# PSilvestre/Clonos

Hardware: AMD Instinct MI355X
Metric: determinants/sec decode+delta-slice (higher is better)
Workload: dtype u8

## Files before the change

### clonos_amd/build.py

```python
from __future__ import annotations

import os
import subprocess
import sys

HERE = os.path.dirname(os.path.abspath(__file__))
ROOT = os.path.dirname(HERE)
CSRC = os.path.join(HERE, "csrc")
LIB = os.path.join(HERE, "libclonos_engine.so")
SOURCES = [os.path.join(CSRC, "engine.cpp"), os.path.join(CSRC, "kernels.hip"), os.path.join(CSRC, "decode_fast.hip"),
           os.path.join(CSRC, "decode_fused.hip"), os.path.join(CSRC, "replay.hip"), os.path.join(CSRC, "encode.hip"),
           os.path.join(CSRC, "response.cpp"), os.path.join(CSRC, "digest.hip"),
           os.path.join(CSRC, "diff.hip")]
HEADERS = [
    os.path.join(CSRC, "kernels.h"),
    os.path.join(CSRC, "jser_device.h"),
    os.path.join(CSRC, "dev_common.h"),
    os.path.join(CSRC, "dev_slow.h"),
    os.path.join(CSRC, "jser_flat.h"),
    os.path.join(CSRC, "handoff.h"),
    os.path.join(CSRC, "digest.h"),
    os.path.join(CSRC, "diff.h"),
    os.path.join(ROOT, "include", "clonos_engine.h"),
]
ARCH = os.environ.get("CLONOS_OFFLOAD_ARCH", "gfx950")


def hipcc() -> str:
    for c in (os.environ.get("HIPCC"), "/opt/rocm/bin/hipcc", "hipcc"):
        if c and (os.path.isabs(c) and os.path.exists(c) or not os.path.isabs(c)):
            return c
    return "hipcc"


def needs_build() -> bool:
    if not os.path.exists(LIB):
        return True
    t = os.path.getmtime(LIB)
    return any(os.path.getmtime(p) > t for p in SOURCES + HEADERS)


def _compile_cmd(src: str, obj: str) -> list:
    return [
        hipcc(),
        "-x", "hip",
        f"--offload-arch={ARCH}",
        "-O3",
        "-std=c++17",
        "-fPIC",
        "-Wall",
        "-Wno-unused-function",
        "-Wno-unused-value",
        "-I", os.path.join(ROOT, "include"),
        "-c", src,
        "-o", obj,
    ]


def build(force: bool = False, verbose: bool = False) -> str:
    if not force and not needs_build():
        return LIB
    hdr_t = max(os.path.getmtime(h) for h in HEADERS)
    objs, procs = [], []
    for src in SOURCES:
        obj = os.path.join(CSRC, os.path.basename(src) + ".o")
        objs.append(obj)
        if not force and os.path.exists(obj) and os.path.getmtime(obj) > max(hdr_t, os.path.getmtime(src)):
            continue
        cmd = _compile_cmd(src, obj)
        if verbose:
            print(" ".join(cmd), flush=True)
        procs.append((src, subprocess.Popen(cmd)))
    bad = [src for src, p in procs if p.wait() != 0]
    if bad:
        raise RuntimeError(f"hipcc failed for {bad}")
    link = [hipcc(), f"--offload-arch={ARCH}", "-shared", "-fPIC", "-o", LIB] + objs
    if verbose:
        print(" ".join(link), flush=True)
    subprocess.run(link, check=True)
    return LIB


if __name__ == "__main__":
    build(force="--force" in sys.argv, verbose=True)
```

### clonos_amd/csrc/engine.cpp

```cpp
#include <hip/hip_runtime.h>
#include <sched.h>

#include <algorithm>
#include <chrono>
#include <condition_variable>
#include <cstdarg>
#include <cstdio>
#include <cstdlib>
#include <cstring>
#include <deque>
#include <functional>
#include <map>
#include <memory>
#include <atomic>
#include <mutex>
#include <string>
#include <thread>
#include <unordered_map>
#include <optional>
#include <vector>

#include "../../include/clonos_engine.h"
#include "diff.h"
#include "digest.h"
#include "kernels.h"

static_assert(sizeof(clg_delta_req) == 32, "clg_delta_req layout");
static_assert(sizeof(clg_diff) == 24, "clg_diff layout");

namespace {

thread_local std::string g_err;

int fail(int code, const char* fmt, ...) {
  char buf[512];
  va_list ap;
  va_start(ap, fmt);
  vsnprintf(buf, sizeof buf, fmt, ap);
  va_end(ap);
  g_err = buf;
  return code;
}

#define HIPCHK(x)                                                                                   \
  do {                                                                                              \
    hipError_t e_ = (x);                                                                            \
    if (e_ != hipSuccess) return fail(CLG_E_DEVICE, "%s failed: %s", #x, hipGetErrorString(e_)); \
  } while (0)

void note_launch_error(const char* what) {
  if (const char* m = clg::take_launch_error()) fail(CLG_E_DEVICE, "%s: %s", what, m);
}
#define CHK(x)                                          \
  do {                                                  \
    int r_ = (x);                                       \
    if (r_ != CLG_OK) {                                 \
      if (r_ == CLG_E_DEVICE) note_launch_error(#x);    \
      return r_;                                        \
    }                                                   \
  } while (0)

struct EpochStart {
  int64_t id;
  int32_t offset;
};
struct Consumer {
  std::shared_ptr<EpochStart> es;
  int32_t offset;
};

template <class T>
struct EpochAlloc {
  using value_type = T;
  EpochAlloc() = default;
  template <class U>
  EpochAlloc(const EpochAlloc<U>&) {}
  struct FreeList : std::vector<void*> {
    ~FreeList() {
      for (void* p : *this) ::operator delete(p);
    }
  };
  static FreeList& free_list() {
    static thread_local FreeList f;
    return f;
  }
  T* allocate(size_t n) {
    auto& f = free_list();
    if (n == 1 && !f.empty()) {
      void* p = f.back();
      f.pop_back();
      return static_cast<T*>(p);
    }
    return static_cast<T*>(::operator new(n * sizeof(T)));
  }
  void deallocate(T* p, size_t n) {
    auto& f = free_list();
    if (n == 1 && f.size() < (1u << 20)) f.push_back(p);
    else ::operator delete(p);
  }
  template <class U>
  bool operator==(const EpochAlloc<U>&) const { return true; }
  template <class U>
  bool operator!=(const EpochAlloc<U>&) const { return false; }
};

struct EpochEnt {
  int64_t id = 0;
  int32_t offset = 0;
  std::shared_ptr<EpochStart> shared;
};
class EpochMap {
 public:
  EpochEnt* begin() { return data(); }
  EpochEnt* end() { return data() + n_; }
  const EpochEnt* begin() const { return data(); }
  const EpochEnt* end() const { return data() + n_; }
  size_t size() const { return n_; }
  bool empty() const { return n_ == 0; }
  EpochEnt* find(int64_t k) {
    EpochEnt* it = lower(k);
    return it != end() && it->id == k ? it : end();
  }
  const EpochEnt* find(int64_t k) const { return const_cast<EpochMap*>(this)->find(k); }
  EpochEnt* emplace(int64_t k, int32_t offset) {
    EpochEnt* it = lower(k);
    if (it != end() && it->id == k) return it;
    const size_t i = size_t(it - begin());
    if (big_.empty() && n_ < kInline) {
      for (size_t j = n_; j > i; --j) inl_[j] = std::move(inl_[j - 1]);
      inl_[i] = EpochEnt{k, offset, nullptr};
    } else {
      if (big_.empty()) {
        big_.reserve(2 * kInline);
        for (uint32_t j = 0; j < n_; ++j) big_.push_back(std::move(inl_[j]));
        for (auto& x : inl_) x.shared.reset();
      }
      big_.insert(big_.begin() + long(i), EpochEnt{k, offset, nullptr});
    }
    ++n_;
    return begin() + i;
  }
  void erase_below(int64_t k) {
    const size_t d = size_t(lower(k) - begin());
    if (!d) return;
    if (big_.empty()) {
      for (size_t j = d; j < n_; ++j) inl_[j - d] = std::move(inl_[j]);
      for (size_t j = n_ - d; j < n_; ++j) inl_[j].shared.reset();
    } else {
      big_.erase(big_.begin(), big_.begin() + long(d));
    }
    n_ -= uint32_t(d);
  }
  void rebase(int32_t move) {
    for (EpochEnt& x : *this) {
      x.offset -= move;
      if (x.shared) x.shared->offset = x.offset;
    }
  }
  static std::shared_ptr<EpochStart> ref(EpochEnt& x) {
    if (!x.shared) x.shared = std::allocate_shared<EpochStart>(EpochAlloc<EpochStart>(), EpochStart{x.id, x.offset});
    return x.shared;
  }

 private:
  static constexpr uint32_t kInline = 2;
  EpochEnt* data() { return big_.empty() ? inl_ : big_.data(); }
  const EpochEnt* data() const { return big_.empty() ? inl_ : big_.data(); }
  EpochEnt* lower(int64_t k) {
    if (n_ == 0 || end()[-1].id < k) return end();
    return std::lower_bound(begin(), end(), k, [](const EpochEnt& a, int64_t b) { return a.id < b; });
  }
  uint32_t n_ = 0;
  EpochEnt inl_[kInline];
  std::vector<EpochEnt> big_;
};

class SegList {
 public:
// ... 154 lines not shown
  ~PinBuf() {
    if (p) hipHostFree(p);
  }
  template <class T>
  T* as() const { return static_cast<T*>(p); }
};

struct Stat {
  uint64_t launches = 0;
  double ms = 0;
  uint64_t bytes = 0;
};
struct PendingTiming {
  std::string name;
  hipEvent_t a, b;
  uint64_t bytes;
};

constexpr size_t kPoolGuard = 256;

constexpr uint32_t kLogStripes = 64;
struct alignas(64) Stripe {
  std::mutex m;
};
struct EngineLock {
  std::mutex m;
  std::atomic<std::thread::id> owner{};
  int depth = 0;
  Stripe stripe[kLogStripes];
  bool owned() const { return owner.load(std::memory_order_relaxed) == std::this_thread::get_id(); }
  void lock() {
    if (owned()) {
      ++depth;
      return;
    }
    m.lock();
    for (auto& s : stripe) s.m.lock();
    owner.store(std::this_thread::get_id(), std::memory_order_relaxed);
    depth = 1;
  }
  void unlock() {
    if (--depth == 0) {
      owner.store(std::thread::id(), std::memory_order_relaxed);
      for (uint32_t i = kLogStripes; i-- > 0;) stripe[i].m.unlock();
      m.unlock();
    }
  }
};
struct XGuard {
  EngineLock& l;
  explicit XGuard(EngineLock& l_) : l(l_) { l.lock(); }
  ~XGuard() { l.unlock(); }
};

class WorkPool {
 public:
  explicit WorkPool(unsigned n) : n_(n ? n : 1) {
    for (unsigned i = 1; i < n_; ++i) th_.emplace_back([this, i] { loop(i); });
  }
  ~WorkPool() {
    {
      std::lock_guard<std::mutex> g(mu_);
      stop_ = true;
    }
    cv_.notify_all();
    for (auto& t : th_) t.join();
  }
  unsigned size() const { return n_; }
  void run(const std::function<void(unsigned, unsigned)>& fn) {
    if (n_ == 1) {
      fn(0, 1);
      return;
    }
    {
      std::lock_guard<std::mutex> g(mu_);
      job_ = &fn;
      left_.store(n_ - 1, std::memory_order_relaxed);
      gen_.fetch_add(1, std::memory_order_release);
    }
    cv_.notify_all();
    fn(0, n_);
    while (left_.load(std::memory_order_acquire) != 0) std::this_thread::yield();
  }

 private:
  void loop(unsigned i) {
    uint64_t seen = 0;
    for (;;) {
      const auto t0 = std::chrono::steady_clock::now();
      while (gen_.load(std::memory_order_acquire) == seen &&
             std::chrono::steady_clock::now() - t0 < std::chrono::microseconds(50))
        std::this_thread::yield();
      const std::function<void(unsigned, unsigned)>* job;
      {
        std::unique_lock<std::mutex> g(mu_);
        cv_.wait(g, [&] { return stop_ || gen_.load(std::memory_order_acquire) != seen; });
        if (stop_) return;
        seen = gen_.load(std::memory_order_acquire);
        job = job_;
      }
      (*job)(i, n_);
      left_.fetch_sub(1, std::memory_order_acq_rel);
    }
  }
  unsigned n_;
  std::vector<std::thread> th_;
  std::mutex mu_;
  std::condition_variable cv_;
  std::atomic<uint64_t> gen_{0};
  std::atomic<unsigned> left_{0};
  const std::function<void(unsigned, unsigned)>* job_ = nullptr;
  bool stop_ = false;
};

}

namespace {
struct Mapped {
  uintptr_t host;
  uint64_t bytes;
  uintptr_t dev;
};
std::mutex g_map_mu;
std::vector<Mapped> g_mapped;
uintptr_t clg_mapped_device_address(const void* h, uint64_t n) {
  std::lock_guard<std::mutex> g(g_map_mu);
  for (const Mapped& m : g_mapped)
    if (uintptr_t(h) >= m.host && uintptr_t(h) < m.host + m.bytes && n <= m.host + m.bytes - uintptr_t(h))
      return m.dev + (uintptr_t(h) - m.host);
  return 0;
}
}

namespace clg_internal {
int set_error(int code, const char* msg) { return fail(code, "%s", msg); }
}

static long long env_num(const char* name, long long dflt, int base = 10) {
  const char* v = getenv(name);
  return v ? strtoll(v, nullptr, base) : dflt;
}
static std::string env_str(const char* name) {
  const char* v = getenv(name);
  return v ? v : "";
}
struct DevSwitches {
  bool robust_decode = env_str("CLONOS_DECODE") == "robust";
  bool small_decode = env_num("CLONOS_SMALL", 1) != 0;
  bool sidecar = env_num("CLONOS_SIDECAR", 1) != 0;
  bool keep_errors = env_num("CLONOS_KEEP_ERRORS", 1) != 0;
  uint32_t fused_perturb = uint32_t(env_num("CLONOS_FUSED_PERTURB", 0, 0));
  size_t jser_arena = getenv("CLONOS_JSER_ARENA") ? std::max<size_t>(256, size_t(env_num("CLONOS_JSER_ARENA", 0, 0))) : 0;
  int gather_prio = int(env_num("CLONOS_GATHER_PRIO", 1));
  int host_threads = int(env_num("CLONOS_HOST_THREADS", 16));
  int lean = int(env_num("CLONOS_LEAN", -1));
  int warm = int(env_num("CLONOS_WARM", -1));
  bool host_prof = getenv("CLONOS_HOST_PROF") != nullptr;
  bool fused_debug = getenv("CLONOS_FUSED_DEBUG") != nullptr;
  bool small_prof = getenv("CLONOS_SMALL_PROF") != nullptr;
  std::string scan_phases = env_str("CLONOS_SCAN_PHASES"), robust_phases = env_str("CLONOS_ROBUST_PHASES"),
              debug_dump = env_str("CLONOS_DEBUG_DUMP");
};

struct clg_engine {
  clg_config cfg{};
  const DevSwitches sw;
  hipStream_t stream = nullptr;
  void* pool_alloc = nullptr;
  uint8_t* pool = nullptr;
  std::vector<uint32_t> free_segs;
  clg::SideCar side{};
  void* side_alloc = nullptr;
  std::vector<uint32_t> seg_life;
  const clg::SideCar* side_arg() const { return side.hdr ? &side : nullptr; }
  uint32_t life_word(uint32_t seg, bool more) const { return (seg_life[seg] & 0x7FFFFFFFu) | (more ? 0x80000000u : 0u); }
  void* ifl_alloc = nullptr;
  uint8_t* ifl_pool = nullptr;
  uint32_t ifl_C = 0;
  std::vector<uint32_t> ifl_free;
  uint8_t* ifl_addr(uint32_t s) const { return ifl_pool + size_t(s) * ifl_C; }
  std::vector<Log> logs;
  std::vector<InFlight> ifls;
  std::map<IdKey, uint32_t> by_id;
  std::vector<Job> jobs;
  std::vector<uint32_t> dirty;
  EngineLock mu;
  std::mutex pool_mu;
  std::mutex dirty_mu;

  PinBuf h_stage, h_desc, h_sres, h_outs;
  static constexpr uint32_t kSlots = 1 + CLG_DECODE_MAX_INFLIGHT;
  PinBuf h_zres_s[kSlots], h_plan_s[kSlots];
  hipEvent_t zdone[kSlots] = {};
  uint32_t plan_slot = 0;
  DevBuf d_stage, d_desc, d_pieces, d_tiles, d_spans, d_agg, d_conv, d_tres, d_sres, d_totals, d_out;
  std::vector<uint64_t> tab_at;
  DevBuf d_fconv, d_lanes, d_sums, d_fres, d_flags, d_dbg, d_prof, d_rprof, d_prof2, d_jpos, d_jlen, d_jn, d_defer;
  DevBuf d_o_off, d_o_tag, d_o_v0, d_o_widx, d_o_wrc, d_o_wv1, d_o_wvo, d_o_wvl, d_o_wsub;
  DevBuf d_zctl, d_ztiles, d_zbits;
  DevBuf d_zjpos, d_zjlen, d_zjn, d_zjwork;
  uint32_t zjovf_cap = 1u << 16;
  uint32_t zjwork_min = 0;
  DevBuf d_zbad;
  DevBuf d_sf_meta, d_sf_rec, d_sf_wide;
  bool jser_hint = false;
  bool lean_hint = true;
  DevBuf d_rmeta, d_rsizes;
  DevBuf d_encin, d_encw, d_encout;
  DevBuf d_hdr;
  DevBuf d_jarena;
  size_t jarena_bytes = size_t(16) << 20;
  PinBuf h_jused;
  hipStream_t gstream = nullptr;
  hipEvent_t gready = nullptr;
  bool g_pending = false;
  PinBuf h_gdesc[2];
  DevBuf d_gdesc[2], d_gpieces[2];
  hipEvent_t gdone[2] = {nullptr, nullptr};
  uint32_t gseq = 0;
  PinBuf h_rmeta;
  PinBuf h_rout;
  DevBuf d_plan;
  DevBuf d_dgtab, d_dgpart, d_dgout;
  PinBuf h_dgout;
  bool dgtab_ready = false;
  DevBuf d_dffirst, d_dfout;
  PinBuf h_dfout;
  bool fused_decode = true;
  bool small_decode = true;

  std::map<std::string, Stat> stats;
  struct HostTimer {
    clg_engine* e;
    const char* name;
    std::chrono::steady_clock::time_point t0;
    HostTimer(clg_engine* en, const char* n) : e(en && en->sw.host_prof ? en : nullptr), name(n) {
      if (e) t0 = std::chrono::steady_clock::now();
    }
    ~HostTimer() {
      if (!e) return;
      Stat& s = e->stats[name];
      s.launches++;
      s.ms += std::chrono::duration<double, std::milli>(std::chrono::steady_clock::now() - t0).count();
    }
    void lap(const char* lap_name) {
      if (!e) return;
      const auto now = std::chrono::steady_clock::now();
      Stat& s = e->stats[lap_name];
      s.launches++;
      s.ms += std::chrono::duration<double, std::milli>(now - t0).count();
      t0 = now;
    }
  };
  std::vector<PendingTiming> timings;
  std::vector<hipEvent_t> ev_pool;

  uint32_t C() const { return cfg.segment_bytes; }
  uint8_t* seg_addr(uint32_t s) const { return pool + size_t(s) * C(); }

  hipEvent_t get_event() {
    if (!ev_pool.empty()) {
      hipEvent_t e = ev_pool.back();
      ev_pool.pop_back();
      return e;
    }
    hipEvent_t e;
    hipEventCreate(&e);
    return e;
  }
  template <class F>
  int timed(const char* name, uint64_t bytes, F&& launch, hipStream_t on = nullptr) {
    if (!(cfg.flags & CLG_F_TIMING)) return launch();
    hipEvent_t a = get_event(), b = get_event();
    hipEventRecord(a, on ? on : stream);
    int r = launch();
    hipEventRecord(b, on ? on : stream);
    timings.push_back(PendingTiming{name, a, b, bytes});
    return r;
  }
  void collect_timings(bool ready_only = false) {
    if (ready_only) {
      std::vector<PendingTiming> later;
      for (auto& t : timings)
        if (hipEventQuery(t.b) == hipErrorNotReady) later.push_back(t);
      if (!later.empty()) {
        std::vector<PendingTiming> done;
        for (auto& t : timings)
          if (hipEventQuery(t.b) != hipErrorNotReady) done.push_back(t);
        timings.swap(done);
        collect_timings();
        timings.swap(later);
        return;
      }
    }
    for (auto& t : timings) {
      float ms = 0;
      hipEventSynchronize(t.b);
      hipEventElapsedTime(&ms, t.a, t.b);
      Stat& s = stats[t.name];
      s.launches++;
      s.ms += ms;
      s.bytes += t.bytes;
      ev_pool.push_back(t.a);
      ev_pool.push_back(t.b);
    }
    timings.clear();
// ... 2657 lines not shown
  std::vector<clg::GatherPiece> pieces;
  runs.reserve(n);
  pieces.reserve(n_pieces);
  uint64_t dst = 0;
  for (uint32_t i = 0; i < n; ++i) {
    if (len[i] == 0) continue;
    runs.push_back(clg::SegSpan{0, 0, uint32_t(len[i]), dst, uint32_t(pieces.size()), i});
    for (uint64_t a = 0; a < len[i]; a += kPiece)
      pieces.push_back(clg::GatherPiece{base + (off[i] - base_off) + a, dst + a, uint32_t(std::min(kPiece, len[i] - a)), 0});
    dst += len[i];
  }
  const size_t rb = clg_engine::al16(runs.size() * sizeof(clg::SegSpan)), pb = pieces.size() * sizeof(clg::GatherPiece);
  CHK(e->h_desc.ensure(rb + pb));
  CHK(e->d_desc.ensure(rb + pb));
  memcpy(e->h_desc.as<uint8_t>(), runs.data(), runs.size() * sizeof(clg::SegSpan));
  memcpy(e->h_desc.as<uint8_t>() + rb, pieces.data(), pb);
  HIPCHK(hipMemcpyAsync(e->d_desc.p, e->h_desc.p, rb + pb, hipMemcpyHostToDevice, e->stream));
  return e->run_digest(e->d_desc.as<clg::SegSpan>(), uint32_t(runs.size()),
                       reinterpret_cast<const clg::GatherPiece*>(e->d_desc.as<uint8_t>() + rb), uint32_t(pieces.size()),
                       total, n, out);
}

int clg_digest_host(const uint8_t* bytes, uint64_t n, clg_digest* out) {
  if (!out || (n && !bytes)) return fail(CLG_E_INVALID_ARG, "null argument");
  *out = clg_digest{clg::dg_bytes(bytes, n), n};
  return CLG_OK;
}

int clg_diff_logs(clg_engine* e, const uint32_t* log, const int64_t* start_epoch, uint32_t n, const uint8_t* bytes,
                  const uint64_t* off, const uint64_t* len, uint32_t in_kind, clg_diff* out) {
  ENGINE_GUARD(e);
  if (n && (!log || !start_epoch || !off || !len || !out)) return fail(CLG_E_INVALID_ARG, "null argument");
  if (in_kind != CLG_MEM_HOST && in_kind != CLG_MEM_DEVICE) return fail(CLG_E_INVALID_ARG, "in_kind %u", in_kind);
  if (!n) return CLG_OK;
  uint64_t lo = UINT64_MAX, hi = 0;
  for (uint32_t i = 0; i < n; ++i) {
    if (len[i] >> 32) return fail(CLG_E_INVALID_ARG, "span %u of %llu bytes", i, (unsigned long long)len[i]);
    if (len[i] == 0) continue;
    lo = std::min(lo, off[i]);
    hi = std::max(hi, off[i] + len[i]);
  }
  if (hi && !bytes) return fail(CLG_E_INVALID_ARG, "null argument");
  std::vector<clg::SegSpan> runs;
  std::vector<uint32_t> segtab, len_log(n);
  uint32_t n_pieces = 0;
  uint64_t total = 0;
  CHK(e->plan_determinant_runs(log, start_epoch, n, len_log.data(), nullptr, runs, segtab, &n_pieces, &total));
  for (uint32_t i = 0; i < n; ++i) out[i] = clg_diff{0, len_log[i], len[i]};
  if (runs.empty()) return CLG_OK;
  CHK(e->flush());
  const uint8_t* base = bytes;
  uint64_t base_off = 0;
  if (in_kind == CLG_MEM_HOST && hi) {
    CHK(e->d_stage.ensure(hi - lo + 16));
    CHK(e->h_stage.ensure(hi - lo + 16));
    memcpy(e->h_stage.p, bytes + lo, hi - lo);
    HIPCHK(hipMemcpyAsync(e->d_stage.p, e->h_stage.p, hi - lo, hipMemcpyHostToDevice, e->stream));
    base = e->d_stage.as<uint8_t>();
    base_off = lo;
  }
  size_t o[2];
  const size_t gb = clg_engine::al16(clg_engine::gather_desc_layout(runs, segtab, o));
  const size_t hb = gb + runs.size() * sizeof(clg::DiffRef);
  CHK(e->h_desc.ensure(hb));
  CHK(e->d_desc.ensure(hb));
  CHK(e->d_pieces.ensure(size_t(n_pieces) * sizeof(clg::GatherPiece)));
  clg_engine::gather_desc_fill(e->h_desc.as<uint8_t>(), runs, segtab, o);
  clg::DiffRef* refs = reinterpret_cast<clg::DiffRef*>(e->h_desc.as<uint8_t>() + gb);
  uint64_t compared = 0;
  for (size_t k = 0; k < runs.size(); ++k) {
    const uint32_t i = runs[k].pad;
    refs[k] = clg::DiffRef{len[i] ? base + (off[i] - base_off) : nullptr, uint32_t(len[i]), 0};
    compared += 2 * std::min<uint64_t>(runs[k].len, len[i]);
  }
  HIPCHK(hipMemcpyAsync(e->d_desc.p, e->h_desc.p, hb, hipMemcpyHostToDevice, e->stream));
  CHK(e->gather_expand(e->d_desc.as<uint8_t>(), runs, o, n_pieces, e->d_pieces.as<clg::GatherPiece>(), e->stream));
  CHK(e->d_dffirst.ensure(size_t(n_pieces) * 4 + 4));
  CHK(e->d_dfout.ensure(size_t(n) * sizeof(clg_diff)));
  CHK(e->h_dfout.ensure(size_t(n) * sizeof(clg_diff)));
  memcpy(e->h_dfout.p, out, size_t(n) * sizeof(clg_diff));
  HIPCHK(hipMemcpyAsync(e->d_dfout.p, e->h_dfout.p, size_t(n) * sizeof(clg_diff), hipMemcpyHostToDevice, e->stream));
  CHK(e->timed("log_diff", compared, [&] {
    return clg::launch_diff(e->d_pieces.as<clg::GatherPiece>(), n_pieces, e->d_desc.as<clg::SegSpan>(),
                            uint32_t(runs.size()), reinterpret_cast<const clg::DiffRef*>(e->d_desc.as<uint8_t>() + gb),
                            e->d_dffirst.as<uint32_t>(), e->d_dfout.as<clg_diff>(), e->stream);
  }));
  HIPCHK(hipMemcpyAsync(e->h_dfout.p, e->d_dfout.p, size_t(n) * sizeof(clg_diff), hipMemcpyDeviceToHost, e->stream));
  CHK(e->sync());
  memcpy(out, e->h_dfout.p, size_t(n) * sizeof(clg_diff));
  return CLG_OK;
}

int clg_lcp_host(const uint8_t* a, uint64_t na, const uint8_t* b, uint64_t nb, uint64_t* lcp) {
  if (!lcp || (na && !a) || (nb && !b)) return fail(CLG_E_INVALID_ARG, "null argument");
  *lcp = clg::df_lcp_bytes(a, na, b, nb);
  return CLG_OK;
}

int clg_slice_batch(clg_engine* e, const clg_slice_req* reqs, uint32_t n, clg_slice_res* res, void* out, uint64_t cap,
                    uint32_t out_kind, uint64_t* total) {
  ENGINE_GUARD_KEEP(e);
  if (!(out_kind == CLG_MEM_DEVICE && (e->cfg.flags & CLG_F_ASYNC_SLICE))) e->settle();
  if (n && (!reqs || !res)) return fail(CLG_E_INVALID_ARG, "null argument");
  CHK(e->flush());
  std::vector<clg::SegSpan> runs;
  std::vector<uint32_t> segtab;
  std::unordered_map<uint32_t, uint64_t> tab_of;
  runs.reserve(n);
  uint32_t n_pieces = 0;
  const uint32_t C = e->C();
  uint64_t dst = 0;
  for (uint32_t i = 0; i < n; ++i) {
    clg_slice_res& r = res[i];
    r = clg_slice_res{CLG_OK, 0, 0, 0, dst};
    const ChKey k{reqs[i].consumer.lo, reqs[i].consumer.hi};
    int32_t has = 0;
    int st = e->has_delta(reqs[i].log, k, reqs[i].epoch, &has);
    if (st != CLG_OK) {
      r.status = st;
      continue;
    }
    r.has_delta = has;
    if (!has) continue;
    st = e->offset_from_epoch(reqs[i].log, k, &r.offset_from_epoch);
    if (st != CLG_OK) {
      r.status = st;
      continue;
    }
    int32_t phys, nb;
    st = e->take_delta(reqs[i].log, k, reqs[i].epoch, &phys, &nb);
    if (st != CLG_OK) {
      r.status = st;
      continue;
    }
    if (dst + uint64_t(nb) > cap) {
      e->logs[reqs[i].log].consumers[k].offset -= nb;
      r.status = CLG_E_CAPACITY;
      continue;
    }
    r.len = nb;
    if (nb > 0) {
      auto ti = tab_of.find(reqs[i].log);
      if (ti == tab_of.end()) {
        const auto& segs = e->logs[reqs[i].log].segs;
        ti = tab_of.emplace(reqs[i].log, segtab.size()).first;
        segtab.insert(segtab.end(), segs.begin(), segs.end());
      }
      runs.push_back(clg::SegSpan{ti->second, uint32_t(phys), uint32_t(nb), dst, n_pieces, 0});
      n_pieces += uint32_t(phys + nb - 1) / C - uint32_t(phys) / C + 1;
    }
    dst += uint64_t(nb);
  }
  if (total) *total = dst;
  return e->run_gather_runs(runs, segtab, n_pieces, dst, out, out_kind);
}

int clg_consumer_seek(clg_engine* e, uint32_t h, clg_channel_id c, int64_t epoch, int32_t offset) {
  ENGINE_GUARD_KEEP(e);
  Log* l;
  CHK(e->get_log(h, &l));
  auto it = l->epochs.find(epoch);
  if (it == l->epochs.end()) return fail(CLG_E_STATE, "epoch %lld not in log", (long long)epoch);
  l->consumers[ChKey{c.lo, c.hi}] = Consumer{EpochMap::ref(*it), offset};
  return CLG_OK;
}

int clg_upstream_delta_batch(clg_engine* e, clg_delta_req* reqs, uint32_t n, const uint8_t* bytes, uint32_t in_kind) {
  ENGINE_GUARD_KEEP(e);
  clg_engine::HostTimer ht(e, "host_abi_upstream");
  e->settle();
  if (n && (!reqs || !bytes)) return fail(CLG_E_INVALID_ARG, "null argument");
  return e->upstream_batch(reqs, n, bytes, in_kind);
}

int clg_consumer_seek_batch(clg_engine* e, const clg_slice_req* reqs, const int32_t* offsets, uint32_t n) {
  ENGINE_GUARD_KEEP(e);
  if (n && (!reqs || !offsets)) return fail(CLG_E_INVALID_ARG, "null argument");
  for (uint32_t i = 0; i < n; ++i) {
    Log* l;
    CHK(e->get_log(reqs[i].log, &l));
    auto it = l->epochs.find(reqs[i].epoch);
    if (it == l->epochs.end()) return fail(CLG_E_STATE, "epoch %lld not in log", (long long)reqs[i].epoch);
    l->consumers[ChKey{reqs[i].consumer.lo, reqs[i].consumer.hi}] = Consumer{EpochMap::ref(*it), offsets[i]};
  }
  return CLG_OK;
}

int clg_truncate_all(clg_engine* e, uint32_t job, int64_t cp, int32_t* applied) {
  ENGINE_GUARD_KEEP(e);
  bool defer = false;
  if (e->any_active()) {
    int64_t mn = INT64_MAX;
    for (const auto& d : e->pq)
      if (d.active) mn = std::min(mn, d.min_epoch);
    const bool dirty = !e->dirty.empty();
    if (cp > mn || dirty) CHK(e->settle());
    else defer = true;
  } else {
    e->release_later();
  }
  if (applied) *applied = 0;
  if (job >= e->jobs.size() || !e->jobs[job].open) return fail(CLG_E_NO_LOG, "unknown job %u", job);
  Job& j = e->jobs[job];
  if (j.latest_cp >= cp) return CLG_OK;
  j.latest_cp = cp;
  ++e->rebase_gen;
  std::vector<uint32_t>& to = defer ? e->free_later : e->free_segs;
  CHK(e->flush());
  clg_engine::HostTimer ht(e, "host_truncate_all");
  if (e->logs.size() >= clg_engine::kParallelLogs) {
    WorkPool* wp = e->workers();
    const unsigned P = wp->size();
    const size_t nl = e->logs.size(), per = (nl + P - 1) / P;
    std::vector<std::vector<uint32_t>> freed(P), later(P);
    std::vector<int> st(P, CLG_OK);
    wp->run([&](unsigned k, unsigned) {
      const size_t i1 = std::min(nl, (k + 1) * per);
      for (size_t i = k * per; i < i1; ++i) {
        if (i + 8 < i1) {
          const char* q = reinterpret_cast<const char*>(&e->logs[i + 8]);
          for (size_t b = 0; b < sizeof(Log); b += 64) __builtin_prefetch(q + b, 1);
        }
        Log& l = e->logs[i];
        if (!l.open || l.job != job) continue;
        bool shared = false;
        for (const EpochEnt& x : l.epochs) {
          if (x.id >= cp) break;
          shared |= x.shared != nullptr;
        }
        if (shared) {
          later[k].push_back(uint32_t(i));
          continue;
        }
        if ((st[k] = e->checkpoint_complete(l, cp, freed[k])) != CLG_OK) return;
      }
    });
    ht.lap("host_trunc_pool");
    for (unsigned k = 0; k < P; ++k) to.insert(to.end(), freed[k].begin(), freed[k].end());
    for (unsigned k = 0; k < P; ++k)
      if (st[k] != CLG_OK) return fail(st[k], "checkpoint completion failed on a log (state outside its bounds)");
    size_t n_later = 0;
    for (unsigned k = 0; k < P; ++k) {
      n_later += later[k].size();
      for (uint32_t i : later[k]) CHK(e->checkpoint_complete(e->logs[i], cp, to));
    }
    ht.lap(n_later ? "host_trunc_later" : "host_trunc_free");
  } else {
    for (auto& l : e->logs)
      if (l.open && l.job == job) CHK(e->checkpoint_complete(l, cp, to));
  }
  if (applied) *applied = 1;
  return CLG_OK;
}

int clg_decode_host(clg_engine* e, const uint8_t* bytes, const uint64_t* span_off, const uint64_t* span_len, uint32_t n,
                    clg_decoded* out, uint64_t* span_rec_base) {
  ENGINE_GUARD(e);
  if (!out || (n && (!span_off || !span_len))) return fail(CLG_E_INVALID_ARG, "null argument");
  uint64_t lo = UINT64_MAX, hi = 0, total = 0;
  for (uint32_t i = 0; i < n; ++i) {
    if (span_len[i] == 0) continue;
    lo = std::min(lo, span_off[i]);
    hi = std::max(hi, span_off[i] + span_len[i]);
    total += span_len[i];
  }
  if (lo == UINT64_MAX) lo = hi = 0;
  CHK(e->d_stage.ensure(hi - lo + 16));
  CHK(e->h_stage.ensure(hi - lo + 16));
  if (hi > lo) {
    memcpy(e->h_stage.p, bytes + lo, hi - lo);
    HIPCHK(hipMemcpyAsync(e->d_stage.p, e->h_stage.p, hi - lo, hipMemcpyHostToDevice, e->stream));
  }
  auto build = [&](clg_engine::DecodePlan& p, uint32_t T) {
    for (uint32_t i = 0; i < n; ++i)
      e->plan_host_span(p, e->d_stage.as<uint8_t>() + (span_len[i] ? span_off[i] - lo : 0), span_len[i], i, T);
  };
  return e->decode(build, total, out, span_rec_base);
}

int clg_decode_logs(clg_engine* e, const uint32_t* log, const int64_t* start_epoch, uint32_t n, clg_decoded* out,
                    uint64_t* span_rec_base) {
  ENGINE_GUARD(e);
  if (!out || (n && (!log || !start_epoch))) return fail(CLG_E_INVALID_ARG, "null argument");
  CHK(e->flush());
  std::vector<int32_t>& st = e->zst;
  std::vector<int32_t>& nb = e->znb;
  st.assign(n, 0);
  nb.assign(n, 0);
  uint64_t total = 0;
  clg_engine::DecodePlan& pf = e->zplan;
  pf.reset();
  if (e->fused_decode) {
    pf.spans.reserve(n);
    pf.runs.reserve(n);
  }
  {
    clg_engine::HostTimer ht(e, "host_decode_plan");
    if (!(n >= clg_engine::kParallelLogs && e->fused_decode && e->plan_parallel(pf, log, start_epoch, n, &total, 0))) {
      total = 0;
      pf.reset();
      for (uint32_t i = 0; i < n; ++i) {
        Log* l;
        CHK(e->get_log(log[i], &l));
        if (l->depth != 0) CHK(e->determinants_range(*l, start_epoch[i], &st[i], &nb[i]));
        total += uint64_t(nb[i]);
        if (e->fused_decode) e->plan_log_span(pf, *l, st[i], nb[i], i, clg::kZTile);
// ... 985 lines not shown
```

### clonos_amd/csrc/kernels.h

```cpp
#pragma once
#include <stddef.h>
#include <stdint.h>

struct clg_digest;
struct clg_diff;

namespace clg {

constexpr int kRegion = 256;
constexpr int kRegions = 64;
constexpr int kTile = kRegion * kRegions;
constexpr int kEntries = 64;

struct TileDesc {
  const uint8_t* abase;
  uint32_t delta;
  uint32_t len;
  uint32_t span;
  uint32_t pad;
  uint64_t span_off;
};

struct SpanDesc {
  uint32_t first_tile;
  uint32_t n_tiles;
  uint64_t len;
};

constexpr uint32_t kExitErr = 0xFFFFFFFFu;
constexpr uint32_t kExitFar = 0xFFFFFFFEu;

struct TileConv {
  uint16_t entry[kRegions];
  uint32_t suffix[kRegions];
  uint32_t exit;
  uint32_t valid;
};

struct TileRes {
  uint32_t entry;
  uint32_t limit;
  uint32_t flags;
  uint32_t pad;
  uint64_t rec_base;
  uint64_t wide_base;
};
constexpr uint32_t kResTableLive = 1;

struct SpanRes {
  uint64_t n_rec;
  uint64_t n_wide;
  int32_t status;
  int32_t err_tag;
  int64_t err_off;
  uint64_t rec_base;
  uint64_t wide_base;
};

struct DecodeOut {
  uint32_t* off;
  uint8_t* tag;
  int64_t* v0;
  uint32_t* w_idx;
  int32_t* w_rc;
  int64_t* w_v1;
  uint32_t* w_var_off;
  uint32_t* w_var_len;
  uint8_t* w_sub;
  uint64_t cap;
  uint64_t wcap;
};

constexpr uint32_t kFRegion = 268;
constexpr int kFOwn = 61;
constexpr int kFNext = 3;
constexpr int kFPoints = kFOwn + kFNext;
constexpr uint32_t kConvUnknown = 0xFFFFFFFFu;

struct LaneSeg {
  uint8_t end;
  uint8_t flags;
  uint16_t far;
  uint32_t cnt;
  uint32_t wcnt;
};
constexpr uint8_t kEndFail = 0xFF;
constexpr uint8_t kEndFar = 0xFE;

struct TileSum {
  uint32_t cnt, wcnt;
  uint8_t f;
  uint8_t x;
  uint16_t far;
  uint32_t pad2;
  uint64_t valid;
};

struct FastRes {
  uint64_t valid;
  uint64_t rec_base;
  uint64_t wide_base;
};

struct JArena {
  uint8_t* base;
  uint64_t cap;
  unsigned long long* used;
};

#ifndef CLG_FCANDS
#define CLG_FCANDS 32
#endif
constexpr int kCands = CLG_FCANDS;
constexpr int kJserCap = 256;

constexpr uint32_t kSideUnknown = 0xFFFFu;
constexpr uint32_t kSideCapMax = 1024;
struct SideCar {
  uint64_t* hdr;
  uint32_t* ent;
  const uint8_t* pool;
  uint64_t pool_bytes;
  uint32_t seg_bytes;
  uint32_t cap;
};

struct JserTabs {
  uint32_t* pos;
  uint32_t* len;
  uint32_t* n;
  uint32_t* defer;
  JArena ar;
  uint64_t* prof = nullptr;
  SideCar side{};
};

int launch_fast_scan(const TileDesc* d_tiles, uint32_t n_tiles, const SpanDesc* d_spans, uint32_t* d_conv, JserTabs J,
                     uint32_t mode, LaneSeg* d_lanes, TileSum* d_sums, uint32_t* d_dbg, uint64_t* d_prof, void* stream);
int launch_jser_fill(const TileDesc* d_tiles, uint32_t n_tiles, const SpanDesc* d_spans, JserTabs J, void* stream);
int launch_fast_resolve(const TileDesc* d_tiles, const SpanDesc* d_spans, uint32_t n_spans, uint32_t* d_conv,
                        LaneSeg* d_lanes, const TileSum* d_sums, JserTabs J, FastRes* d_fres, SpanRes* d_sres,
                        uint32_t* d_span_flags, JArena ar, void* stream);
int launch_fast_emit(const TileDesc* d_tiles, uint32_t n_tiles, const SpanDesc* d_spans, const uint32_t* d_conv,
                     JserTabs J, const LaneSeg* d_lanes, const FastRes* d_fres, const SpanRes* d_sres,
                     const uint32_t* d_span_flags, DecodeOut out, void* stream);

constexpr uint32_t kZRegion = 128;
constexpr uint32_t kZTile = 64 * kZRegion;
constexpr uint32_t kZHalo = 64;

enum ZAbort : uint32_t {
  kZAbortNone = 0,
  kZAbortAny = 0,
  kZAbortBad = 1,
  kZAbortEnd = 2,
// ... 59 lines not shown
constexpr uint32_t kZDbgWalkGaveUp = 0xD15A;
constexpr uint32_t kZDbgLaneWords = 8;
constexpr uint32_t kZDbgTiles = kZDbgLanes + 64 * kZDbgLaneWords;

struct FusedCtl {
  uint64_t* st_x;
  uint64_t* cnt;
  uint64_t* base;
  uint64_t* boff;
  uint64_t* bits;
  uint64_t* span_lo;
  uint64_t* span_hi;
  uint32_t* abort;
  uint32_t* dbg;
  uint64_t* prof;
  uint32_t n_tiles;
  uint32_t* jpos;
  uint32_t* jlen;
  uint32_t* jn;
  uint32_t jser;
  uint32_t jwork_cap;
  uint32_t* jwork;
  uint32_t warm;
  JArena jar;
  uint32_t* span_bad;
  uint32_t skip_bad;
  const uint32_t* chunk;
  uint32_t tiny;
  uint64_t* ex;
  uint8_t* rep_flag;
  uint32_t* rep;
  uint64_t* ent;
  uint32_t perturb;
  uint32_t lb_check;
  uint32_t n_spans;
  uint64_t* span_err;
  uint32_t* jbase;
  uint32_t jovf_cap;
  uint64_t* lb;
  uint64_t* h_res;
  uint32_t lean;
  SideCar side;
};
constexpr uint32_t kZScanBlock = 1024;
static_assert(sizeof(FusedCtl) == 328, "the kernels' argument layout: no field added, resized or moved");

struct FusedLayout {
  size_t ex, rep_flag, cnt, base, boff, span_lo, span_hi, abort, lb, ent, words;
};
inline FusedLayout fused_layout(uint32_t n_tiles, uint32_t n_spans, uint32_t grid) {
  const size_t nt = n_tiles, ns = n_spans, nb = (nt + kZScanBlock - 1) / kZScanBlock;
  FusedLayout L;
  L.ex = nt;
  L.rep_flag = L.ex + nt;
  L.cnt = L.rep_flag + (nt + 7) / 8;
  L.base = L.cnt + nt;
  L.boff = L.base + nt;
  L.span_lo = L.boff + nb;
  L.span_hi = L.span_lo + ns;
  L.abort = L.span_hi + ns;
  L.lb = L.abort + kZAbortWords / 2;
  L.ent = L.lb + 1 + nb;
  L.words = L.ent + (grid ? grid : 1);
  return L;
}
struct FusedReadback {
  uint32_t span_hi;
  uint64_t abort, abort_only, jwork, words;
};
constexpr FusedReadback fused_readback(uint32_t n_spans) {
  return FusedReadback{n_spans, 2ull * n_spans, 2ull * n_spans + kZAbortFlagWords / 2,
                       2ull * n_spans + kZHabJWork / 2, 2ull * n_spans + (kZHabJWork + kZJWorkHead) / 2};
}
constexpr uint32_t kZJCap = 256;
constexpr uint32_t kZTinySpan = 1024;
enum class FusedPhase : uint32_t {
  Count = 0,
  Scan3 = 1,
  Emit = 2,
  JserTables = 3,
  CountTiny = 4,
  Scan = 5,
};
int launch_decode_inject(const SpanDesc* d_spans, const uint32_t* d_bad, const uint64_t* d_packed, uint32_t n_bad,
                         FusedCtl ctl, void* stream);
int launch_add_u32(uint32_t* d_x, uint64_t n, uint32_t delta, void* stream);
struct SfPlace {
  uint64_t rbase, nrec, wbase, nwide;
  uint32_t span, pad;
};
int launch_sf_place(const SfPlace* d_place, uint32_t n_bad, DecodeOut scratch, DecodeOut out, FusedCtl ctl, void* stream);
int launch_err_classify(const TileDesc* d_tiles, const SpanDesc* d_spans, const uint32_t* d_bad, uint32_t n_bad,
                        FusedCtl ctl, int32_t* d_res, JArena ar, void* stream);
int launch_decode_fused(const TileDesc* d_tiles, uint32_t n_tiles, const SpanDesc* d_spans, uint32_t n_spans,
                        FusedCtl ctl, DecodeOut out, void* stream, FusedPhase phase);
uint32_t decode_count_grid(bool jser, uint32_t n_tiles);

constexpr uint32_t kZSmallSpans = 4096;
constexpr uint32_t kZSmallTilesMax = 4096;
constexpr uint32_t kZSmallAggWords = 2 * kZSmallTilesMax;
constexpr uint32_t kZSmallArgTiles = 64, kZSmallArgSpans = 64;
enum ZSmallRes : uint32_t {
  kZSmallRec = 0,
  kZSmallWide = 1,
  kZSmallFailed = 2,
  kZSmallSpan0 = 3,
};
enum ZSmallCheck : uint32_t {
  kZCheckEntryExit = 0,
  kZCheckBase = 1,
  kZCheckCount = 2,
};
constexpr uint32_t kZSmallCheckWords = 3;
constexpr uint64_t small_check_at(uint32_t n_spans, uint32_t t) {
  return uint64_t(kZSmallSpan0) + n_spans + uint64_t(kZSmallCheckWords) * t;
}
constexpr uint64_t small_res_words(uint32_t n_spans, uint32_t n_tiles) { return small_check_at(n_spans, n_tiles); }
struct SmallPlanArg {
  TileDesc tiles[kZSmallArgTiles];
  SpanDesc spans[kZSmallArgSpans];
};
int launch_decode_small(const TileDesc* d_tiles, uint32_t n_tiles, const SpanDesc* d_spans, uint32_t n_spans,
                        FusedCtl ctl, DecodeOut out, uint64_t* agg, uint64_t* agg_next, uint64_t* res, void* stream,
                        const SmallPlanArg* plan = nullptr);

struct GatherPiece {
  const uint8_t* src;
  uint64_t dst;
  uint32_t len;
  uint32_t pad;
};

constexpr uint32_t kDigestTabWin = 32, kDigestTabOne = kDigestTabWin + 64, kDigestTabIter = kDigestTabOne + 9,
                   kDigestTabWords = kDigestTabIter + 1;
void digest_table(uint64_t* tab);
int launch_digest(const GatherPiece* d_pieces, uint32_t n_pieces, const struct SegSpan* d_runs, uint32_t n_runs,
                  const uint64_t* d_tab, uint64_t* d_partial, ::clg_digest* d_out, void* stream);

struct DiffRef {
  const uint8_t* ref;
  uint32_t len;
  uint32_t pad;
};
int launch_diff(const GatherPiece* d_pieces, uint32_t n_pieces, const struct SegSpan* d_runs, uint32_t n_runs,
                const DiffRef* d_refs, uint32_t* d_first, ::clg_diff* d_out, void* stream);

struct ScatterChunk {
  uint8_t* dst;
  uint64_t src;
  uint32_t len;
  uint32_t life;
};

struct SegSpan {
  uint64_t segtab_off;
  uint32_t phys;
  uint32_t len;
  uint64_t dst;
  uint32_t first;
  uint32_t pad;
};
int launch_status(hipError_t e);
const char* take_launch_error();
int launch_expand_pieces(const SegSpan* d_spans, uint32_t n_spans, uint32_t n_pieces, const uint32_t* d_segtab,
                         const uint8_t* pool, uint32_t seg_bytes, GatherPiece* d_out, void* stream);
int launch_expand_tiles(const SegSpan* d_spans, uint32_t n_spans, uint32_t n_tiles, const uint32_t* d_segtab,
                        const uint8_t* pool, uint32_t seg_bytes, uint32_t unit, TileDesc* d_out, void* stream);
constexpr int kPrepRanges = 8;
struct PrepRange {
  uint32_t* dst;
  const uint32_t* src;
  uint64_t n;
  uint32_t val;
  uint32_t pad;
};
struct PrepArgs {
  const SegSpan* runs;
  uint32_t n_runs, n_tiles;
  const uint32_t* segtab;
  const uint8_t* pool;
  uint32_t C, U;
  TileDesc* tiles;
  uint64_t total;
  PrepRange r[kPrepRanges];
};
int launch_decode_prep(PrepArgs a, void* stream);

int launch_scatter(const ScatterChunk* d_chunks, uint32_t n, const uint8_t* d_src, void* stream,
                   const SideCar* side = nullptr);
int launch_gather(const GatherPiece* d_pieces, uint32_t n, uint8_t* d_out, void* stream);
int launch_decode_tables(const TileDesc* d_tiles, uint32_t n_tiles, const SpanDesc* d_spans,
                         uint64_t* d_agg, TileConv* d_conv, const uint32_t* d_span_flags, JArena ar, void* stream);
int launch_decode_resolve(const TileDesc* d_tiles, const SpanDesc* d_spans, uint32_t n_spans,
                          const uint64_t* d_agg, const TileConv* d_conv, TileRes* d_tres,
                          SpanRes* d_sres, const uint32_t* d_span_flags, JArena ar, void* stream);
int launch_decode_spanscan(SpanRes* d_sres, uint32_t n_spans, uint64_t* d_totals, void* stream);
int launch_decode_emit(const TileDesc* d_tiles, uint32_t n_tiles, const SpanDesc* d_spans,
                       const TileConv* d_conv, const TileRes* d_tres, const SpanRes* d_sres,
                       const uint32_t* d_span_flags, DecodeOut out, JArena ar, void* stream);


struct EncodeIn {
  const uint8_t* tag;
  const int64_t* v0;
  const uint32_t* w_idx;
  const int32_t* w_rc;
  const int64_t* w_v1;
  const uint32_t* w_var_off;
  const uint32_t* w_var_len;
  const uint8_t* w_sub;
  const uint8_t* var;
  uint64_t n, n_wide;
};
int launch_encode(const EncodeIn& in, uint32_t* d_wsum, uint64_t* d_wbase, uint64_t* d_bsum, uint64_t* d_bbase,
                  uint32_t* d_bad, uint8_t* d_out, uint32_t phase, void* stream);

struct BufSpan {
  const uint8_t* src;
  uint64_t len;
  uint64_t out_base;
};
struct BufChunk {
  uint32_t span;
  uint32_t pad;
  uint64_t k0, k1;
};
int launch_bufsizes(const BufChunk* d_chunks, uint32_t n_chunks, const BufSpan* d_spans, int32_t* d_sizes,
                    uint64_t* d_first_bad, void* stream);
int launch_bufsizes_classify(const BufSpan* d_spans, uint32_t n_spans, const uint64_t* d_first_bad,
                             uint64_t* d_count, int32_t* d_status, int64_t* d_err_off, int32_t* d_err_tag,
                             JArena ar, void* stream);

}
```

Before: 88.62 billion.

## Reorder gather runs by log and physical window to improve source locality

Before launching the gather for consumer reads, the run list is regrouped by log (segment table offset). Each log's runs are split into fixed-size physical windows and emitted window by window, so reads from the same region of a log's segments are issued close together. The intent is better cache and TLB locality on the source pool when requests interleave logs. The cost is host-side sorting and splitting, plus extra sub-spans and pieces when runs cross window boundaries.

```diff
diff --git a/clonos_amd/build.py b/clonos_amd/build.py
--- a/clonos_amd/build.py
+++ b/clonos_amd/build.py
@@ -19,6 +19,7 @@
     os.path.join(CSRC, "dev_slow.h"),
     os.path.join(CSRC, "jser_flat.h"),
     os.path.join(CSRC, "handoff.h"),
+    os.path.join(CSRC, "slice_order.h"),
     os.path.join(CSRC, "digest.h"),
     os.path.join(CSRC, "diff.h"),
     os.path.join(ROOT, "include", "clonos_engine.h"),
diff --git a/clonos_amd/csrc/engine.cpp b/clonos_amd/csrc/engine.cpp
--- a/clonos_amd/csrc/engine.cpp
+++ b/clonos_amd/csrc/engine.cpp
@@ -24,6 +24,7 @@
 #include "diff.h"
 #include "digest.h"
 #include "kernels.h"
+#include "slice_order.h"
 
 static_assert(sizeof(clg_delta_req) == 32, "clg_delta_req layout");
 static_assert(sizeof(clg_diff) == 24, "clg_diff layout");
@@ -484,6 +485,7 @@
   uint32_t fused_perturb = uint32_t(env_num("CLONOS_FUSED_PERTURB", 0, 0));
   size_t jser_arena = getenv("CLONOS_JSER_ARENA") ? std::max<size_t>(256, size_t(env_num("CLONOS_JSER_ARENA", 0, 0))) : 0;
   int gather_prio = int(env_num("CLONOS_GATHER_PRIO", 1));
+  long long gather_window = env_num("CLONOS_GATHER_WINDOW", -1);
   int host_threads = int(env_num("CLONOS_HOST_THREADS", 16));
   int lean = int(env_num("CLONOS_LEAN", -1));
   int warm = int(env_num("CLONOS_WARM", -1));
@@ -3447,6 +3449,8 @@
     dst += uint64_t(nb);
   }
   if (total) *total = dst;
+  const long long gw = e->sw.gather_window;
+  clg::window_order(runs, C, gw < 0 ? clg::default_window(C) : uint32_t(std::min<long long>(gw, UINT32_MAX)));
   return e->run_gather_runs(runs, segtab, n_pieces, dst, out, out_kind);
 }
 
diff --git a/clonos_amd/csrc/kernels.h b/clonos_amd/csrc/kernels.h
--- a/clonos_amd/csrc/kernels.h
+++ b/clonos_amd/csrc/kernels.h
@@ -1,6 +1,8 @@
 #pragma once
 #include <stddef.h>
 #include <stdint.h>
+
+#include "slice_order.h"
 
 struct clg_digest;
 struct clg_diff;
@@ -366,14 +368,6 @@
   uint32_t life;
 };
 
-struct SegSpan {
-  uint64_t segtab_off;
-  uint32_t phys;
-  uint32_t len;
-  uint64_t dst;
-  uint32_t first;
-  uint32_t pad;
-};
 int launch_status(hipError_t e);
 const char* take_launch_error();
 int launch_expand_pieces(const SegSpan* d_spans, uint32_t n_spans, uint32_t n_pieces, const uint32_t* d_segtab,
diff --git a/clonos_amd/csrc/slice_order.h b/clonos_amd/csrc/slice_order.h
--- /dev/null
+++ b/clonos_amd/csrc/slice_order.h
@@ -0,0 +1,70 @@
+#pragma once
+#include <stdint.h>
+
+#include <algorithm>
+#include <vector>
+
+namespace clg {
+
+struct SegSpan {
+  uint64_t segtab_off;
+  uint32_t phys;
+  uint32_t len;
+  uint64_t dst;
+  uint32_t first;
+  uint32_t pad;
+};
+
+constexpr uint32_t kGatherWindowBytes = 2u << 20;
+constexpr uint32_t default_window(uint32_t C) { return C && C < kGatherWindowBytes ? kGatherWindowBytes / C : 1u; }
+
+inline uint32_t span_pieces(const SegSpan& r, uint32_t C) { return (r.phys + r.len - 1) / C - r.phys / C + 1; }
+
+inline bool window_order(std::vector<SegSpan>& runs, uint32_t C, uint32_t W) {
+  const size_t n = runs.size();
+  if (!W || !C || n < 2) return false;
+  size_t i = 1;
+  for (uint64_t top = runs[0].segtab_off; i < n && runs[i].segtab_off > top; ++i) top = runs[i].segtab_off;
+  if (i == n) return false;
+  std::vector<uint64_t> keys;
+  std::vector<uint32_t> grp(n), at;
+  for (size_t k = 0; k < n; ++k) {
+    const uint64_t key = runs[k].segtab_off;
+    if (keys.empty() || key > keys.back()) keys.push_back(key);
+    grp[k] = uint32_t(std::lower_bound(keys.begin(), keys.end(), key) - keys.begin());
+  }
+  at.assign(keys.size() + 1, 0);
+  for (size_t k = 0; k < n; ++k) ++at[grp[k] + 1];
+  for (size_t g = 0; g < keys.size(); ++g) at[g + 1] += at[g];
+  std::vector<uint32_t> by_log(n);
+  {
+    std::vector<uint32_t> fill(at.begin(), at.end() - 1);
+    for (size_t k = 0; k < n; ++k) by_log[fill[grp[k]]++] = uint32_t(k);
+  }
+  const uint64_t win = uint64_t(W) * C;
+  std::vector<SegSpan> out;
+  out.reserve(n * 2);
+  uint32_t first = 0;
+  for (size_t g = 0; g < keys.size(); ++g) {
+    uint64_t w0 = UINT64_MAX, w1 = 0;
+    for (uint32_t j = at[g]; j < at[g + 1]; ++j) {
+      const SegSpan& r = runs[by_log[j]];
+      w0 = std::min(w0, r.phys / win);
+      w1 = std::max(w1, (uint64_t(r.phys) + r.len - 1) / win);
+    }
+    for (uint64_t w = w0; w <= w1; ++w) {
+      for (uint32_t j = at[g]; j < at[g + 1]; ++j) {
+        const SegSpan& r = runs[by_log[j]];
+        const uint64_t s = std::max<uint64_t>(r.phys, w * win), e = std::min(uint64_t(r.phys) + r.len, (w + 1) * win);
+        if (s >= e) continue;
+        SegSpan sub{r.segtab_off, uint32_t(s), uint32_t(e - s), r.dst + (s - r.phys), first, r.pad};
+        first += span_pieces(sub, C);
+        out.push_back(sub);
+      }
+    }
+  }
+  runs.swap(out);
+  return true;
+}
+
+}
```

Measured after the change: 90.16 billion (median of 6 runs). +1.7%, better.
